# ScottHCL/recommend

Hardware: AMD Instinct MI355X
Metric: ranked samples/sec (fwd+bwd) at B=4096 seq=128; AUC parity vs ref (higher is better)
Workload: dtype f32-emulated (fp16-pair / split-bf16); 1 GPU; C2: OneTrans 4L d128 H4 f512 L_NS12 L_S128 (seq 3x42), Criteo-shape 13 dense + 26 ids, replicated tables, fwd+bwd+optimizer; global_batch=4096, per_gpu_batch=4096, seq_len=128, parallelism=dp1

## Files before the change

include/onetrans_hip.h:

```cpp
#ifndef ONETRANS_HIP_H
#define ONETRANS_HIP_H

#include <stddef.h>
#include <stdint.h>

#ifdef __cplusplus
extern "C" {
#endif

#define OT_OK 0
#define OT_ERR_INVALID_ARG 1
#define OT_ERR_UNSUPPORTED 2
#define OT_ERR_HIP 3

#define OT_GEMM_NN 0
#define OT_GEMM_NT 1

#define OT_AX_NONE 0
#define OT_AX_RMSNORM 1
#define OT_AX_GELU 2
#define OT_AX_BF16 4
#define OT_AX_BF16_RMSNORM 5

#define OT_EPI_BIAS 1
// ... 73 lines not shown
                           float* dW, int64_t dw_gstride, float* db, int64_t db_gstride,
                           int accumulate, void* workspace, size_t ws_bytes, const float* a_bound,
                           const float* d_bound, int precision, void* stream);

int ot_transpose_banks(const float* src, float* dst, const int64_t* banks_dev, int nbanks, int64_t total_tiles,
                       void* stream);

size_t ot_split_image_elems(int G, int N, int K);
int ot_split_images(const float* base, const int64_t* desc_dev, int ndesc, int64_t total_units, uint16_t* img,
                    int precision, void* stream);
int ot_mixed_gemm_img(int mode, const float* A, int64_t lda, int K, const int32_t* in_rows,
                      int a_xform, const float* a_rstd, const float* a_gamma,
                      const float* W, int64_t w_gstride, int64_t ldw, int N,
                      const int32_t* tile_group, int ntiles,
                      const float* bias, int64_t bias_gstride,
                      float* C, int64_t ldc, const int32_t* out_rows, int epi,
                      const float* res, int64_t ldres, int res_tok,
                      const float* aux, int64_t ldaux,
                      uint32_t seed, uint32_t site, float drop_rate, int tail_K, int tail_I,
                      const int32_t* tail_pos, const uint16_t* b_image, int image_ntn, int image_tn0,
                      int precision, void* stream);
int ot_plane_wide(int on);
int ot_wgrad_wide(int on);
int ot_mixed_gemm_rms_img(int mode, const float* A, int64_t lda, int K, const int32_t* in_rows,
                          int a_xform, const float* a_rstd, const float* a_gamma,
                          const float* W, int64_t w_gstride, int64_t ldw, int N,
                          const int32_t* tile_group, int ntiles,
                          const float* bias, int64_t bias_gstride,
                          float* C, int64_t ldc, const int32_t* out_rows, int epi,
                          const float* res, int64_t ldres, int res_tok,
                          const float* aux, int64_t ldaux,
                          uint32_t seed, uint32_t site, float drop_rate, int tail_K, int tail_I,
                          const int32_t* tail_pos, const ot_rms_epilogue* rms, const uint16_t* b_image,
                          int image_ntn, int image_tn0, int precision, void* stream);

int ot_attn_fwd(const float* qkv, int64_t ld, int B, int H, int I, int K, const int32_t* qpos,
                int head_dim, float* out, float* lse, int precision, void* stream);
size_t ot_attn_fwd_fp8_workspace_size(int B, int H, int I, int head_dim);
int ot_attn_fwd_fp8(const float* qkv, int64_t ld, int B, int H, int I, int K, const int32_t* qpos,
                    int head_dim, float* out, float* lse, void* workspace, size_t ws_bytes, void* stream);
#define OT_FP8_DEQUANT 1
#define OT_FP8_TWO_TERM 2
int ot_attn_fwd_fp8_ex(float* qkv, int64_t ld, int B, int H, int I, int K, const int32_t* qpos, int head_dim,
                       float* out, float* lse, void* workspace, size_t ws_bytes, int flags, void* stream);
int ot_attn_fwd_fp8_deq16(const float* qkv, int64_t ld, int B, int H, int I, int K, const int32_t* qpos,
                          int head_dim, float* out, float* lse, void* workspace, size_t ws_bytes, int flags,
// ... 135 lines not shown
```

recommend_amd/_lib.py:

```python

from __future__ import annotations

import ctypes
import os
from ctypes import c_float, c_int, c_int64, c_size_t, c_uint32, c_void_p, c_char_p

_HERE = os.path.dirname(os.path.abspath(__file__))
LIB_PATH = os.environ.get('ONETRANS_HIP_LIB') or os.path.join(_HERE, 'libonetrans_hip.so')
HEADER = os.path.join(os.path.dirname(_HERE), 'include', 'onetrans_hip.h')

OT_GEMM_NN, OT_GEMM_NT = 0, 1
OT_AX_NONE, OT_AX_RMSNORM, OT_AX_GELU, OT_AX_BF16, OT_AX_BF16_RMSNORM = 0, 1, 2, 4, 5
OT_EPI_BIAS, OT_EPI_GELU_BWD, OT_EPI_GELU = 1, 2, 4
OT_EPI_DROPOUT, OT_EPI_RESIDUAL, OT_EPI_ACCUMULATE = 8, 16, 32
OT_EPI_ROW_RSTD, OT_EPI_RMSNORM_BWD, OT_EPI_ROWDOT = 64, 128, 256
OT_EPI_C_BF16 = 512
OT_EPI_AUX_BF16 = 1024
OT_ATTN_DQKV_BF16 = 1
OT_ATTN_QKV_BF16 = 2
OT_ATTN_DQ_PART_BF16 = 4
OT_WG_D_BF16 = 8
OT_MATMUL_F32, OT_MATMUL_SPLIT_BF16, OT_MATMUL_BF16 = 0, 1, 2
OT_FP8_DEQUANT, OT_FP8_TWO_TERM = 1, 2
MATMUL_MODES = {'f32': OT_MATMUL_F32, 'split': OT_MATMUL_SPLIT_BF16, 'bf16': OT_MATMUL_BF16}
# ... 24 lines not shown
    'ot_gemm_tile_rows': (c_int, []),
    'ot_mixed_gemm': (c_int, [c_int, P, I64, c_int, P, c_int, P, P, P, I64, I64, c_int, P, c_int, P, I64,
                              P, I64, P, c_int, P, I64, c_int, P, I64, c_uint32, c_uint32, c_float, c_int,
                              c_int, P, c_int, P]),
    'ot_mixed_gemm_rms_workspace_size': (c_size_t, [c_int, c_int]),
    'ot_mixed_gemm_rms': (c_int, [c_int, P, I64, c_int, P, c_int, P, P, P, I64, I64, c_int, P, c_int, P, I64,
                                  P, I64, P, c_int, P, I64, c_int, P, I64, c_uint32, c_uint32, c_float, c_int,
                                  c_int, P, P, c_int, P]),
    'ot_wgrad_workspace_size': (c_size_t, [c_int, c_int, c_int]),
    'ot_mixed_gemm_wgrad': (c_int, [P, I64, P, c_int, P, P, P, I64, P, c_int, c_int, P, c_int, P, c_int, P,
                                    I64, P, I64, c_int, P, c_size_t, c_int, P]),
    'ot_mixed_gemm_wgrad_ex': (c_int, [P, I64, P, c_int, P, P, P, I64, P, c_int, c_int, P, c_int, P, c_int, P,
                                       I64, P, I64, c_int, P, c_size_t, P, P, c_int, P]),
    'ot_transpose_banks': (c_int, [P, P, P, c_int, I64, P]),
    'ot_mixed_gemm_img': (c_int, [c_int, P, I64, c_int, P, c_int, P, P, P, I64, I64, c_int, P, c_int, P, I64,
                                  P, I64, P, c_int, P, I64, c_int, P, I64, c_uint32, c_uint32, c_float, c_int,
                                  c_int, P, P, c_int, c_int, c_int, P]),
    'ot_mixed_gemm_rms_img': (c_int, [c_int, P, I64, c_int, P, c_int, P, P, P, I64, I64, c_int, P, c_int, P, I64,
                                      P, I64, P, c_int, P, I64, c_int, P, I64, c_uint32, c_uint32, c_float, c_int,
                                      c_int, P, P, P, c_int, c_int, c_int, P]),
    'ot_split_image_elems': (c_size_t, [c_int, c_int, c_int]),
    'ot_plane_wide': (c_int, [c_int]),
    'ot_wgrad_wide': (c_int, [c_int]),
    'ot_split_images': (c_int, [P, P, c_int, I64, P, c_int, P]),
    'ot_attn_fwd': (c_int, [P, I64, c_int, c_int, c_int, c_int, P, c_int, P, P, c_int, P]),
    'ot_attn_fwd_fp8_workspace_size': (c_size_t, [c_int, c_int, c_int, c_int]),
    'ot_attn_fwd_fp8': (c_int, [P, I64, c_int, c_int, c_int, c_int, P, c_int, P, P, P, c_size_t, P]),
    'ot_attn_fwd_fp8_ex': (c_int, [P, I64, c_int, c_int, c_int, c_int, P, c_int, P, P, P, c_size_t, c_int, P]),
    'ot_attn_fwd_fp8_deq16': (c_int, [P, I64, c_int, c_int, c_int, c_int, P, c_int, P, P, P, c_size_t, c_int, P, P]),
    'ot_attn_bwd_workspace_size': (c_size_t, [c_int, c_int, c_int]),
    'ot_attn_bwd': (c_int, [P, I64, P, P, P, c_int, c_int, c_int, c_int, P, c_int, P, P, c_int, P]),
    'ot_attn_bwd_ex_workspace_size': (c_size_t, [c_int, c_int, c_int, c_int, c_int, c_int, c_int]),
    'ot_attn_bwd_ex': (c_int, [P, I64, P, P, P, c_int, c_int, c_int, c_int, P, c_int, P, P, c_size_t, c_int, P]),
    'ot_attn_bwd_dqkv_bf16_supported': (c_int, [c_int, c_int, c_int, c_int, c_int]),
    'ot_attn_bwd_bf16_forms': (c_int, [c_int, c_int, c_int, c_int, c_int]),
    'ot_attn_slice_supported': (c_int, [c_int, c_int, c_int, c_int]),
    'ot_attn_bwd_flags_workspace_size': (c_size_t, [c_int, c_int, c_int, c_int, c_int, c_int, c_int, c_int]),
    'ot_attn_bwd_flags': (c_int, [P, I64, P, P, P, c_int, c_int, c_int, c_int, P, c_int, P, c_int, P, c_size_t, c_int, P]),
    'ot_attn_fwd_cached': (c_int, [P, I64, P, I64, P, c_int, c_int, c_int, c_int, c_int, c_int, P, P]),
    'ot_attn_amax_supported': (c_int, [c_int, c_int, c_int, c_int, c_int]),
    'ot_attn_fwd_amax': (c_int, [P, I64, c_int, c_int, c_int, c_int, P, c_int, P, P, P, P, c_int, P]),
    'ot_attn_bwd_amax': (c_int, [P, I64, P, P, P, c_int, c_int, c_int, c_int, P, c_int, P, P, c_size_t, P, P, c_int,
                                 P]),
    'ot_pyramid_select': (c_int, [P, c_float, c_int, c_int, c_int, c_int, P, P, P, c_int, P]),
    'ot_rmsnorm_fwd': (c_int, [P, I64, P, P, I64, P, I64, c_int, c_float, P]),
    'ot_rmsnorm_bwd_workspace_size': (c_size_t, [I64, c_int]),
# ... 89 lines not shown
```

recommend_amd/csrc/gemm.hip:

```cpp
#include <algorithm>
#include <cstdlib>
#include <atomic>
#include <mutex>

#include "common.h"

namespace ot {

#ifndef OT_GEMM_BK
#define OT_GEMM_BK 16
#endif
#ifndef OT_GEMM_MINWG
#define OT_GEMM_MINWG 3
#endif
#ifndef OT_GEMM_PRIO
#define OT_GEMM_PRIO 0
#endif
#ifndef OT_GEMM_RMS_EARLY
#define OT_GEMM_RMS_EARLY 1
#endif
#ifndef OT_PLANE_BF16_NSTG
#define OT_PLANE_BF16_NSTG 3
#endif
constexpr int PLANE_BF16_NSTG = OT_PLANE_BF16_NSTG;
// ... 33 lines not shown
  const int32_t* tile_group;
  const float* bias; int64_t bias_gstride;
  float* C; int64_t ldc; const int32_t* out_rows;
  int epi;
  const float* res; int64_t ldres; int res_tok;
  const float* aux; int64_t ldaux;
  uint32_t seed, site, drop_thr; float drop_scale; int tail_K, tail_I; int drop_width;
  int ntm, ntn;
  float* rstd_out; float eps;
  const float* nx; int64_t ldnx; const float* ngamma; const float* nrstd;
  const float* dres; int64_t lddres; int dres_K, dres_I; const int32_t* dres_inv;
  float* dxm; int64_t lddxm; float* dgpart;
  float* rowpart;
  float* rowdot; int rowdot_n;
  uint16_t* gelu_out; int64_t ldgelu;
  const int32_t* tail_pos;
  const uint16_t* bimg; int bimg_ntn, bimg_tn0;
  uint16_t* xn_out; int64_t ldxn;
  uint16_t* c16_out; int64_t ldc16;
  float* rowmax_out; int rowmax_n;
  const float* a_rowmax; int a_rowmax_n;
  float* amax_out;
  float* rowabs_out; int rowabs_n;
};

__device__ __forceinline__ float row32_max(float v) {
  v = fmaxf(v, __int_as_float(__builtin_amdgcn_update_dpp(0, __float_as_int(v), 0xB1, 0xF, 0xF, false)));
  v = fmaxf(v, __int_as_float(__builtin_amdgcn_update_dpp(0, __float_as_int(v), 0x4E, 0xF, 0xF, false)));
  v = fmaxf(v, __int_as_float(__builtin_amdgcn_update_dpp(0, __float_as_int(v), 0x141, 0xF, 0xF, false)));
  v = fmaxf(v, __int_as_float(__builtin_amdgcn_update_dpp(0, __float_as_int(v), 0x140, 0xF, 0xF, false)));
  const auto a = __builtin_amdgcn_permlane16_swap(__float_as_uint(v), __float_as_uint(v), false, false);
  return fmaxf(__uint_as_float(a[0]), __uint_as_float(a[1]));
}
__device__ __forceinline__ float row32_sum(float v) {
#pragma unroll
  for (int o = 16; o > 0; o >>= 1) v += __shfl_xor(v, o, 64);
  return v;
}

__device__ __forceinline__ f32x4 apply_pro(f32x4 v, int xf, float rs, const float* gamma, int k) {
  if (xf == OT_AX_RMSNORM) {
    v.x *= rs * gamma[k]; v.y *= rs * gamma[k + 1]; v.z *= rs * gamma[k + 2]; v.w *= rs * gamma[k + 3];
  } else if (xf == OT_AX_GELU) {
    v = gelu_erf4(v);
  }
  return v;
// ... 9 lines not shown
    rem = b % per_chunk;
    return true;
  }
  const int x = b & 7, j = b >> 3;
  c = x + 8 * (j / per_chunk);
  rem = j % per_chunk;
  return c < nchunks;
}

__device__ __forceinline__ void store_out4(float* dst, f32x4 v) {
  if (OT_GEMM_NT_STORE) __builtin_nontemporal_store(v, reinterpret_cast<f32x4*>(dst));
  else *reinterpret_cast<f32x4*>(dst) = v;
}
#ifndef OT_GEMM_NT_STORE16
#define OT_GEMM_NT_STORE16 1
#endif
__device__ __forceinline__ void store_out4_bf16(uint16_t* dst, f32x4 v) {
  if (OT_GEMM_NT_STORE16) __builtin_nontemporal_store(bf16_rne4(v), reinterpret_cast<u32x2*>(dst));
  else *reinterpret_cast<u32x2*>(dst) = bf16_rne4(v);
}

template <int EPIT, int LAYOUT, bool ROWSCALE, int RBN = 8, bool GS = false>
__device__ __forceinline__ void gemm_vec_epilogue(const GemmArgs& p, const f32x16* acc, float* smem, int tm,
                                                  int n0, int g, int sub = 0, int tid = -1) {
  const int epi = EPIT;
  const int t = tid >= 0 ? tid : (int)threadIdx.x, lane = t & 63, wave = t >> 6;
  const int h = lane >> 5, li = lane & 31;
    constexpr int CLD = GT + 4;
    static_assert(64 * CLD + 8 * GT <= 4 * GT * GLD, "epilogue LDS exceeds the staging buffers");
    float* ct = smem;
    const int c4 = t & 31, rb = t >> 5;
    const int col = n0 + 4 * c4;
    f32x4 bias4 = {0.f, 0.f, 0.f, 0.f};
    if (epi & OT_EPI_BIAS) bias4 = *reinterpret_cast<const f32x4*>(p.bias + (int64_t)g * p.bias_gstride + col);
    const bool need_tok = (epi & OT_EPI_DROPOUT) || ((epi & OT_EPI_RESIDUAL) && p.res_tok);
    constexpr bool RMSBWD = EPIT >= 0 && (EPIT & OT_EPI_RMSNORM_BWD);
    constexpr bool ROWRSTD = EPIT >= 0 && (EPIT & OT_EPI_ROW_RSTD);
    constexpr bool ROWDOT = EPIT >= 0 && (EPIT & OT_EPI_ROWDOT);
    constexpr bool GSTORE = GS && (EPIT == OT_EPI_BIAS || EPIT == (OT_EPI_BIAS | OT_EPI_C_BF16));
    constexpr bool CBF = EPIT >= 0 && (EPIT & OT_EPI_C_BF16);
    constexpr bool AUXBF = EPIT >= 0 && (EPIT & OT_EPI_AUX_BF16);
    f32x4 rdb4 = {0.f, 0.f, 0.f, 0.f};
    if (ROWDOT) rdb4 = *reinterpret_cast<const f32x4*>(p.bias + (int64_t)g * p.bias_gstride + col);
    float* dgs = ct + 64 * CLD;
    f32x4 ngam = {0.f, 0.f, 0.f, 0.f};
    if (RMSBWD) {
      ngam = *reinterpret_cast<const f32x4*>(p.ngamma + col);
      *reinterpret_cast<f32x4*>(dgs + rb * GT + 4 * c4) = f32x4{0.f, 0.f, 0.f, 0.f};
    }
    constexpr int RB = RMSBWD ? RBN / 2 : RBN;
    float am = 0.f;
#pragma unroll
    for (int hf = 0; hf < 2; ++hf) {
      int orow[8];
      float rsc[8];
#pragma unroll
      for (int i = 0; i < 8; ++i) {
        const int lr = rb + 8 * i;
        const int64_t gr = (int64_t)tm * GT + (LAYOUT == 0 ? (lr >> 5) * 64 + 32 * hf + (lr & 31) : 64 * hf + lr);
        orow[i] = p.out_rows ? p.out_rows[gr] : (int)gr;
        if (ROWSCALE) {
          const int ir = p.in_rows ? p.in_rows[gr] : (int)gr;
          rsc[i] = ir >= 0 ? p.a_rstd[ir] : 0.f;
        }
      }
      if (LAYOUT == 0) {
#pragma unroll
        for (int n = 0; n < 2; ++n)
#pragma unroll
          for (int r = 0; r < 16; ++r)
            ct[((wave >> 1) * 32 + (r & 3) + 8 * (r >> 2) + 4 * h) * CLD + (wave & 1) * 64 + 32 * n + li] = acc[2 * hf + n][r];
      } else if (LAYOUT == 1) {
        if ((wave >> 1) == hf) {
#pragma unroll
          for (int nb = 0; nb < 4; ++nb)
#pragma unroll
            for (int r = 0; r < 16; ++r)
              ct[((wave & 1) * 32 + (r & 3) + 8 * (r >> 2) + 4 * h) * CLD + 32 * nb + li] = acc[nb][r];
        }
      } else if (LAYOUT == 4) {
        if ((wave >> 1) == sub) {
#pragma unroll
// ... 489 lines not shown
        }
        crow[col] = v;
      }
    }
  }
}

__global__ __launch_bounds__(256) void row_rstd_finish_kernel(const float* __restrict__ part, int ntn,
                                                              const int32_t* __restrict__ out_rows, int64_t nrows,
                                                              int N, float eps, float* rstd_out) {
  const int64_t gr = (int64_t)blockIdx.x * blockDim.x + threadIdx.x;
  if (gr >= nrows) return;
  const int orr = out_rows ? out_rows[gr] : (int)gr;
  if (orr < 0) return;
  float s = 0.f;
  for (int j = 0; j < ntn; ++j) s += part[gr * ntn + j];
  rstd_out[orr] = rsqrtf(s / (float)N + eps);
}

constexpr int PG_A_BYTES = GT * 16 * 4;
constexpr int PG_B_BYTES = 3 * GT * 16 * 2;
constexpr int PG_STG_BYTES = PG_A_BYTES + PG_B_BYTES;
static_assert(64 * (GT + 4) * 4 + 8 * GT * 4 <= 2 * PG_STG_BYTES, "plane GEMM epilogue LDS");

typedef __attribute__((address_space(3))) void lds_void_t;

template <int TERMS>
constexpr int pg_stage_bytes() { return PG_A_BYTES + (TERMS == 1 ? GT * 16 * 2 : PG_B_BYTES); }

constexpr uint32_t PAIR_IMAGE_TAG = 0x7FC17FC1u;

template <int AXT, int EPIT, int NSTG, int MINW, int TERMS = 6>
__global__ __launch_bounds__(256, MINW) void plane_gemm_kernel(GemmArgs p) {
  static_assert(NSTG >= 2 && NSTG <= 4, "plane GEMM stages");
  static_assert(TERMS == 6 || TERMS == 1 || (TERMS == 2 && (AXT == OT_AX_RMSNORM || AXT == OT_AX_GELU || AXT == OT_AX_NONE)),
                "plane GEMM terms");
  constexpr bool ABF = AXT == OT_AX_BF16 || AXT == OT_AX_BF16_RMSNORM;
  constexpr bool RSC = AXT == OT_AX_RMSNORM || AXT == OT_AX_BF16_RMSNORM;
  static_assert(!ABF || TERMS == 1, "bf16 A operands go with OT_MATMUL_BF16");
  constexpr int STG = pg_stage_bytes<TERMS>();
  extern __shared__ __attribute__((aligned(16))) float smem[];
  char* lds = reinterpret_cast<char*>(smem);
  const int nwg = p.ntm * p.ntn;
  const int wg = xcd_remap(blockIdx.x, nwg);
  const int tm = wg / p.ntn, tn = wg % p.ntn;
  const int g = p.tile_group ? p.tile_group[tm] : 0;
// ... 57 lines not shown
  const int aoff0 = ra * 64 + 16 * ((2 * h) ^ ((li >> 2) & 3));
  const int aoff1 = ra * 64 + 16 * ((2 * h + 1) ^ ((li >> 2) & 3));
  const int boff = PG_A_BYTES + li * 32 + 16 * (h ^ ((li >> 3) & 1));
  const int aoffb = ra * 32 + 16 * (h ^ ((li >> 3) & 1));

  bool xnw = false;
  float xrs = 0.f;
  uint16_t* xnp = nullptr;
  float* gsm = reinterpret_cast<float*>(lds + NSTG * STG);
  constexpr bool XN = RSC && TERMS == 1;
  if (XN && p.xn_out && tn == 0) {
    for (int k = 4 * t; k < p.K; k += 4 * 256)
      *reinterpret_cast<f32x4*>(gsm + k) = *reinterpret_cast<const f32x4*>(p.a_gamma + k);
    const int64_t xgr = (int64_t)tm * GT + ra;
    const int xir = p.in_rows ? p.in_rows[xgr] : (int)xgr;
    xnw = xir >= 0;
    if (xnw) {
      xrs = p.a_rstd[xir];
      xnp = p.xn_out + (int64_t)xir * p.ldxn + 8 * h;
    }
  }

  float abound = 1.f;
  if constexpr (TERMS == 2) {
    const int64_t gr = (int64_t)tm * GT + ra;
    int ir = p.in_rows ? p.in_rows[gr] : (int)gr;
    ir = ir < 0 ? 0 : ir;
    if constexpr (AXT == OT_AX_RMSNORM) {
      abound = p.a_rstd[ir];
    } else {
      abound = AXT == OT_AX_GELU ? 0.17f : 0.f;
      for (int j = 0; j < p.a_rowmax_n; ++j) abound = fmaxf(abound, p.a_rowmax[(int64_t)ir * p.a_rowmax_n + j]);
    }
  }
  issue(0, 0);
  if (NSTG >= 3 && nk > 1) issue(1, 1);
  if (NSTG >= 4 && nk > 2) issue(2, 2);
  float asc = 1.f, ainv = 1.f;
  if constexpr (TERMS == 2) {
    asc = pow2_scale14(AXT == OT_AX_RMSNORM ? sqrtf((float)p.K) / abound : abound);
    ainv = 1.f / asc;
  }
  for (int kt = 0; kt < nk; ++kt) {
    constexpr int OPS = ABF ? 2 : (TERMS == 1 ? 3 : 2 + BPL);
    const int ahead = (NSTG - 2 < nk - 1 - kt) ? NSTG - 2 : nk - 1 - kt;
    if (ahead >= 2) asm volatile("s_waitcnt vmcnt(%0)" :: "n"(2 * OPS) : "memory");
    else if (ahead == 1) asm volatile("s_waitcnt vmcnt(%0)" :: "n"(OPS) : "memory");
    else asm volatile("s_waitcnt vmcnt(0)" ::: "memory");
    asm volatile("s_waitcnt lgkmcnt(0)" ::: "memory");
    __builtin_amdgcn_s_barrier();
    asm volatile("" ::: "memory");
    if (kt + NSTG - 1 < nk) issue(kt + NSTG - 1, (kt + NSTG - 1) % NSTG);
    const char* sb = lds + (kt % NSTG) * STG;
    u32x4 fb[4][3];
#pragma unroll
    for (int nb = 0; nb < 4; ++nb)
#pragma unroll
      for (int q = 0; q < (TERMS == 1 ? 1 : BPL); ++q)
        fb[nb][q] = *reinterpret_cast<const u32x4*>(sb + boff + q * 4096 + nb * 1024);
    if constexpr (ABF) {
      u32x4 fa[3];
      fa[0] = *reinterpret_cast<const u32x4*>(sb + aoffb);
      if (XN && xnw) {
        const float* gp = gsm + 16 * kt + 8 * h;
// ... 31 lines not shown
#pragma unroll
      for (int nb = 0; nb < 4; ++nb) acc[nb] = mfma_pair(fa, fb[nb], acc[nb]);
    } else {
      split8t<TERMS == 1 ? 1 : 6>(av, fa);
#pragma unroll
      for (int nb = 0; nb < 4; ++nb) acc[nb] = mfma_terms<TERMS == 1 ? 1 : 6>(fa, fb[nb], acc[nb]);
    }
  }
  if constexpr (TERMS == 2) {
    const float* csc = reinterpret_cast<const float*>(bimg0 + 2 * GT * 16 * 2);
    const float bad = reinterpret_cast<const uint32_t*>(csc)[GT] == PAIR_IMAGE_TAG ? 1.f : __builtin_nanf("");
    float cinv[4];
#pragma unroll
    for (int nb = 0; nb < 4; ++nb) cinv[nb] = bad / csc[32 * nb + li];
#pragma unroll
    for (int r = 0; r < 16; ++r) {
      const float ri = __shfl(ainv, (r & 3) + 8 * (r >> 2) + 4 * h, 64);
#pragma unroll
      for (int nb = 0; nb < 4; ++nb) acc[nb][r] *= ri * cinv[nb];
    }
  }
  asm volatile("s_waitcnt vmcnt(0) lgkmcnt(0)" ::: "memory");
  __syncthreads();
  gemm_vec_epilogue<EPIT, 1, RSC, MINW >= 4 ? OT_PLANE_EPI_RBN : 8, TERMS == 1>(p, acc, smem, tm, n0, g);
}

#ifndef OT_PLANE_WIDE
#define OT_PLANE_WIDE 1
#endif
#ifndef OT_PLANE_WIDE_WL
#define OT_PLANE_WIDE_WL 2
#endif
constexpr int PW_COLS = 2 * GT;
template <int AXT>
constexpr bool pw_abf() { return AXT == OT_AX_BF16 || AXT == OT_AX_BF16_RMSNORM; }
template <int AXT>
constexpr int pw_abytes() { return pw_abf<AXT>() ? GT * 32 : GT * 64; }
template <int AXT>
constexpr int pw_sub() { return pw_abytes<AXT>() + 2 * GT * 32; }
template <int AXT>
constexpr int pw_nstg() { return pw_abf<AXT>() ? 3 : 2; }
template <int AXT>
constexpr int pw_stage_lds() { return pw_nstg<AXT>() * 2 * pw_sub<AXT>(); }

template <int AXT, int EPIT, int WL = OT_PLANE_WIDE_WL>
__global__ __launch_bounds__(256, 2) void plane_wide_kernel(GemmArgs p) {
  static_assert(AXT == OT_AX_NONE || pw_abf<AXT>(), "wide plane GEMM: A in f32 (rounded) or bf16");
// ... 491 lines not shown
  X(OT_AX_BF16_RMSNORM, 0)                                                                     \
  X(OT_AX_BF16_RMSNORM, OT_EPI_BIAS)                                                           \
  X(OT_AX_BF16_RMSNORM, OT_EPI_BIAS | OT_EPI_C_BF16)                                           \
  X(OT_AX_BF16, 0)                                                                             \
  X(OT_AX_BF16, OT_EPI_BIAS | OT_EPI_RESIDUAL)                                                 \
  X(OT_AX_BF16, OT_EPI_BIAS | OT_EPI_RESIDUAL | OT_EPI_DROPOUT)                                \
  X(OT_AX_BF16, OT_EPI_BIAS | OT_EPI_RESIDUAL | OT_EPI_DROPOUT | OT_EPI_ROW_RSTD)              \
  X(OT_AX_BF16, OT_EPI_BIAS | OT_EPI_RESIDUAL | OT_EPI_ROW_RSTD)                               \
  X(OT_AX_BF16, OT_EPI_GELU_BWD | OT_EPI_ROWDOT | OT_EPI_C_BF16 | OT_EPI_AUX_BF16)             \
  X(OT_AX_BF16, OT_EPI_GELU_BWD | OT_EPI_ROWDOT | OT_EPI_C_BF16)                               \
  X(OT_AX_BF16, OT_EPI_RMSNORM_BWD | OT_EPI_DROPOUT)                                           \
  X(OT_AX_BF16, OT_EPI_RMSNORM_BWD)

static int plane_tile_auto(int K, int N, int ntiles) {
  (void)ntiles;
  return N <= K ? 1 : 0;
}

static std::atomic<int> g_plane_wide{OT_PLANE_WIDE};
extern "C" int ot_plane_wide(int on) {
  const int prev = g_plane_wide.load();
  if (on >= 0) g_plane_wide.store(on > 4 ? 4 : on);
  return prev;
}

static void (*plane_wide_for(int x, int e, int kind, int* stage_lds))(GemmArgs) {
  void (*k)(GemmArgs) = nullptr;
#define OT_WIDE_PICK(AX_, EP_)                                                                        \
  if (x == (AX_) && e == (EP_)) {                                                                     \
    k = kind == 3 ? plane_sq_kernel<AX_, EP_> : kind == 2 ? plane_big_kernel<AX_, EP_> : plane_wide_kernel<AX_, EP_>; \
    *stage_lds = kind == 3 ? ps_stage_lds<AX_>() : kind == 2 ? pb_stage_lds<AX_>() : pw_stage_lds<AX_>();  \
  }
  OT_WIDE_LIST(OT_WIDE_PICK)
#undef OT_WIDE_PICK
  static std::once_flag once;
  std::call_once(once, [] {
#define OT_WIDE_ATTR(AX_, EP_)                                                                               \
  (void)hipFuncSetAttribute((const void*)plane_wide_kernel<AX_, EP_>, hipFuncAttributeMaxDynamicSharedMemorySize, \
                            pw_stage_lds<AX_>() + 4096);                                                         \
  (void)hipFuncSetAttribute((const void*)plane_big_kernel<AX_, EP_>, hipFuncAttributeMaxDynamicSharedMemorySize,  \
                            pb_stage_lds<AX_>() + 4096);                                                        \
  (void)hipFuncSetAttribute((const void*)plane_sq_kernel<AX_, EP_>, hipFuncAttributeMaxDynamicSharedMemorySize,   \
                            ps_stage_lds<AX_>() + 4096);
    OT_WIDE_LIST(OT_WIDE_ATTR)
#undef OT_WIDE_ATTR
    (void)hipGetLastError();
// ... 1206 lines not shown
      p.dgpart = dgpart;
    }
  }
  if (epi & OT_EPI_DROPOUT) {
    OT_REQUIRE(drop_rate >= 0.f && drop_rate < 1.f, "ot_mixed_gemm: drop_rate out of range");
    p.drop_thr = drop_threshold(drop_rate);
    p.drop_scale = 1.f / (1.f - drop_rate);
  }
  const bool split = prec != OT_MATMUL_F32 && mode == OT_GEMM_NT;
  const bool one = prec == OT_MATMUL_BF16;
  const size_t shmem = split ? 4 * GT * SRS * sizeof(uint16_t) : 4 * GT * GLD * sizeof(float);
  auto a16 = [](const void* q) { return ((uintptr_t)q & 15) == 0; };
  const bool vec_ok = ldc % 4 == 0 && a16(C) && (!(epi & OT_EPI_RESIDUAL) || (ldres % 4 == 0 && a16(res))) &&
                      (!(epi & OT_EPI_GELU_BWD) || (ldaux % 4 == 0 && a16(aux))) &&
                      (!(epi & (OT_EPI_BIAS | OT_EPI_ROWDOT)) || (bias_gstride % 4 == 0 && a16(bias)));
  const bool edge = (K % GBK) != 0 || (N % GT) != 0 || !vec_ok;
  OT_REQUIRE(!rms_flags || !edge, "ot_mixed_gemm_rms: needs K %% %d == 0 and 16-B aligned operands", GBK);
  const unsigned nwg = (unsigned)ntiles * p.ntn;
  hipStream_t s = (hipStream_t)stream;
  void (*kern)(GemmArgs) = nullptr;
  bool plane = false;
  int wide_lds = 0;
  int wide_kind = 0;
  const int e = epi, x = a_xform;
#define OT_SPEC(NT_, AX_, EP_)                                                                  \
  if (mode == (NT_ ? OT_GEMM_NT : OT_GEMM_NN) && x == AX_ && e == (EP_))                         \
    kern = split ? (one ? (edge ? mixed_gemm_kernel<NT_, AX_, EP_, true, 1> : mixed_gemm_kernel<NT_, AX_, EP_, false, 1>) \
                        : (edge ? mixed_gemm_kernel<NT_, AX_, EP_, true, SPLIT_TERMS>                         \
                                : mixed_gemm_kernel<NT_, AX_, EP_, false, SPLIT_TERMS>))                      \
                 : (edge ? mixed_gemm_kernel<NT_, AX_, EP_, true, 0> : mixed_gemm_kernel<NT_, AX_, EP_, false, 0>);
  OT_SPEC(true, OT_AX_RMSNORM, 0)
  OT_SPEC(true, OT_AX_RMSNORM, OT_EPI_BIAS)
  OT_SPEC(true, OT_AX_GELU, OT_EPI_BIAS | OT_EPI_RESIDUAL | OT_EPI_DROPOUT)
  OT_SPEC(true, OT_AX_GELU, OT_EPI_BIAS | OT_EPI_RESIDUAL)
  OT_SPEC(true, OT_AX_NONE, OT_EPI_RESIDUAL | OT_EPI_DROPOUT)
  OT_SPEC(true, OT_AX_NONE, OT_EPI_RESIDUAL)
  OT_SPEC(true, OT_AX_NONE, OT_EPI_BIAS)
  OT_SPEC(true, OT_AX_NONE, OT_EPI_GELU_BWD)
  OT_SPEC(true, OT_AX_NONE, OT_EPI_GELU_BWD | OT_EPI_ROWDOT)
  OT_SPEC(true, OT_AX_NONE, 0)
  OT_SPEC(true, OT_AX_NONE, OT_EPI_ACCUMULATE)
  OT_SPEC(true, OT_AX_NONE, OT_EPI_RESIDUAL | OT_EPI_DROPOUT | OT_EPI_ROW_RSTD)
  OT_SPEC(true, OT_AX_NONE, OT_EPI_RESIDUAL | OT_EPI_ROW_RSTD)
  OT_SPEC(true, OT_AX_GELU, OT_EPI_BIAS | OT_EPI_RESIDUAL | OT_EPI_DROPOUT | OT_EPI_ROW_RSTD)
  OT_SPEC(true, OT_AX_GELU, OT_EPI_BIAS | OT_EPI_RESIDUAL | OT_EPI_ROW_RSTD)
  OT_SPEC(true, OT_AX_NONE, OT_EPI_RMSNORM_BWD)
// ... 36 lines not shown
    if (one && x == OT_AX_NONE && e == (OT_EPI_GELU_BWD | OT_EPI_C_BF16 | OT_EPI_AUX_BF16))
      pk = plane_gemm_kernel<OT_AX_NONE, OT_EPI_GELU_BWD | OT_EPI_C_BF16 | OT_EPI_AUX_BF16, PLANE_BF16_NSTG, 4, 1>;
    if (one && x == OT_AX_NONE && e == (OT_EPI_GELU_BWD | OT_EPI_ROWDOT | OT_EPI_AUX_BF16))
      pk = plane_gemm_kernel<OT_AX_NONE, OT_EPI_GELU_BWD | OT_EPI_ROWDOT | OT_EPI_AUX_BF16, PLANE_BF16_NSTG, 4, 1>;
    if (one && x == OT_AX_RMSNORM && e == (OT_EPI_BIAS | OT_EPI_C_BF16))
      pk = plane_gemm_kernel<OT_AX_RMSNORM, OT_EPI_BIAS | OT_EPI_C_BF16, PLANE_BF16_NSTG, 4, 1>;
#define OT_PSPEC_BF(EP_) if (one && x == OT_AX_BF16 && e == (EP_)) pk = plane_gemm_kernel<OT_AX_BF16, EP_, PLANE_BF16_NSTG, 4, 1>;
    OT_PSPEC_BF(OT_EPI_BIAS | OT_EPI_RESIDUAL | OT_EPI_DROPOUT)
    OT_PSPEC_BF(OT_EPI_BIAS | OT_EPI_RESIDUAL)
    OT_PSPEC_BF(OT_EPI_BIAS | OT_EPI_RESIDUAL | OT_EPI_DROPOUT | OT_EPI_ROW_RSTD)
    OT_PSPEC_BF(OT_EPI_BIAS | OT_EPI_RESIDUAL | OT_EPI_ROW_RSTD)
    OT_PSPEC_BF(OT_EPI_RMSNORM_BWD)
    OT_PSPEC_BF(OT_EPI_RMSNORM_BWD | OT_EPI_DROPOUT)
    OT_PSPEC_BF(0)
    OT_PSPEC_BF(OT_EPI_GELU_BWD | OT_EPI_ROWDOT | OT_EPI_C_BF16 | OT_EPI_AUX_BF16)
    OT_PSPEC_BF(OT_EPI_GELU_BWD | OT_EPI_ROWDOT | OT_EPI_C_BF16)
#undef OT_PSPEC_BF
#define OT_PSPEC_BR(EP_) if (one && x == OT_AX_BF16_RMSNORM && e == (EP_)) pk = plane_gemm_kernel<OT_AX_BF16_RMSNORM, EP_, PLANE_BF16_NSTG, 4, 1>;
    OT_PSPEC_BR(0)
    OT_PSPEC_BR(OT_EPI_BIAS)
    OT_PSPEC_BR(OT_EPI_BIAS | OT_EPI_C_BF16)
#undef OT_PSPEC_BR
    if (pk) { kern = pk; plane = true; }
    const int wmode = g_plane_wide.load(std::memory_order_relaxed);
    if (pk && one && wmode && N % PW_COLS == 0 && K % 32 == 0 && !(p.xn_out && K > 1024)) {
      int kind = wmode == 1 ? plane_tile_auto(K, N, ntiles) : wmode - 1;
      if (kind == 2 && N % PB_COLS != 0) kind = 1;
      if (kind == 3 && ntiles % 2 != 0) kind = 1;
      int stage_lds = 0;
      void (*wk)(GemmArgs) = kind ? plane_wide_for(x, e, kind, &stage_lds) : nullptr;
      if (wk) {
        kern = wk;
        wide_lds = stage_lds;
        wide_kind = kind;
      }
    }
  }
  OT_REQUIRE((x != OT_AX_BF16 && x != OT_AX_BF16_RMSNORM) || plane,
             "ot_mixed_gemm: no plane GEMM for a_xform %d with epilogue %d (or edge tiles)", x, epi);
  OT_REQUIRE(!p.c16_out || (plane && one && p.ldc16 % 4 == 0 && ((uintptr_t)p.c16_out % 8) == 0 &&
                            !(epi & (OT_EPI_RMSNORM_BWD | OT_EPI_C_BF16))),
             "ot_mixed_gemm_rms: c16_out needs the bf16-mode plane GEMM (not with OT_EPI_RMSNORM_BWD / C_BF16), "
             "ldc16 %% 4 == 0 and 8-B alignment");
  OT_REQUIRE(!(epi & (OT_EPI_C_BF16 | OT_EPI_AUX_BF16)) || plane,
             "ot_mixed_gemm: OT_EPI_C_BF16 / OT_EPI_AUX_BF16 need the bf16-mode plane GEMM with OT_EPI_GELU_BWD "
             "[| OT_EPI_ROWDOT] or OT_EPI_BIAS alone (epilogue %d)", epi);
// ... 27 lines not shown
    else if (mode == OT_GEMM_NT && split)
      kern = edge ? mixed_gemm_kernel<true, -1, -1, true, SPLIT_TERMS> : mixed_gemm_kernel<true, -1, -1, false, SPLIT_TERMS>;
    else if (mode == OT_GEMM_NT)
      kern = edge ? mixed_gemm_kernel<true, -1, -1, true, 0> : mixed_gemm_kernel<true, -1, -1, false, 0>;
    else
      kern = edge ? mixed_gemm_kernel<false, -1, -1, true, 0> : mixed_gemm_kernel<false, -1, -1, false, 0>;
  }
  static std::once_flag lds_once;
  std::call_once(lds_once, [] {
    const int bytes = (int)std::max(4 * GT * GLD * sizeof(float), 4 * GT * SRS * sizeof(uint16_t));
    for (void (*k)(GemmArgs) : {mixed_gemm_kernel<true, -1, -1, true, 0>, mixed_gemm_kernel<true, -1, -1, false, 0>,
                                mixed_gemm_kernel<false, -1, -1, true, 0>, mixed_gemm_kernel<false, -1, -1, false, 0>,
                                mixed_gemm_kernel<true, -1, -1, true, SPLIT_TERMS>,
                                mixed_gemm_kernel<true, -1, -1, false, SPLIT_TERMS>,
                                mixed_gemm_kernel<true, -1, -1, true, 1>, mixed_gemm_kernel<true, -1, -1, false, 1>})
      (void)hipFuncSetAttribute((const void*)k, hipFuncAttributeMaxDynamicSharedMemorySize, bytes);
    (void)hipGetLastError();
  });
  if (wide_lds > 0) {
    const size_t wshm = std::max((size_t)wide_lds + xn_lds, (size_t)(64 * (GT + 4) + 8 * GT) * 4);
    const unsigned wg = wide_kind == 3 ? (unsigned)(ntiles / 2) * (unsigned)(N / PW_COLS)
                                       : (unsigned)ntiles * (unsigned)(N / (wide_kind == 2 ? PB_COLS : PW_COLS));
    hipLaunchKernelGGL(kern, dim3(wg), dim3(wide_kind == 3 ? 512 : 256), wshm, s, p);
  } else {
    hipLaunchKernelGGL(kern, dim3(nwg), dim3(256), launch_shmem, s, p);
  }
  OT_LAUNCH_CHECK("ot_mixed_gemm");
  if (dgpart) {
    launch_colsum_reduce(dgpart, ntiles, N, rms->dgamma, rms->accumulate_dgamma, s, dgpart + (int64_t)ntiles * N);
    OT_LAUNCH_CHECK("ot_mixed_gemm_rms(dgamma)");
  }
  if (p.rowpart) {
    const int64_t nr = (int64_t)ntiles * GT;
    hipLaunchKernelGGL(row_rstd_finish_kernel, dim3(ceil_div(nr, 256)), dim3(256), 0, s, p.rowpart, p.ntn, out_rows,
                       nr, N, rms->eps, rms->rstd_out);
    OT_LAUNCH_CHECK("ot_mixed_gemm_rms(rstd)");
  }
  return OT_OK;
}

extern "C" int ot_mixed_gemm(int mode, const float* A, int64_t lda, int K, const int32_t* in_rows,
                             int a_xform, const float* a_rstd, const float* a_gamma,
                             const float* W, int64_t w_gstride, int64_t ldw, int N,
                             const int32_t* tile_group, int ntiles,
                             const float* bias, int64_t bias_gstride,
                             float* C, int64_t ldc, const int32_t* out_rows, int epi,
// ... 236 lines not shown
```

recommend_amd/kernels.py:

```python

from __future__ import annotations

import contextlib
import ctypes
import functools
import os
import threading
from typing import Optional, Tuple, Union

import torch

from . import _lib
from ._lib import call, size

Ptrish = Union[None, torch.Tensor, Tuple[torch.Tensor, int]]


class Probe:

    def __init__(self):
        self.recs = []

    def begin(self):
        ev = torch.cuda.Event(enable_timing=True)
# ... 249 lines not shown
        _probe.end('mixed_gemm', 2.0 * m_rows * K * N, ev, f'wgrad ax{a_xform} M{m_rows} K{K} N{N} ch{nchunks}',
                   (2.0 if (a_xform & ~_lib.OT_WG_D_BF16) == _lib.OT_AX_BF16 else 4.0) * m_rows * K
                   + (2.0 if a_xform & _lib.OT_WG_D_BF16 else 4.0) * m_rows * N
                   + 4.0 * m_rows * ((a_xform & ~_lib.OT_WG_D_BF16) == _lib.OT_AX_RMSNORM) + 4.0 * ngroups * K * N,
                   wterms)


def transpose_banks(src, dst, banks_dev, nbanks, total_tiles) -> None:
    call('ot_transpose_banks', ptr(src), ptr(dst), ptr(banks_dev), nbanks, total_tiles, stream())


def split_image_elems(G: int, N: int, K: int) -> int:
    return int(_lib.load().ot_split_image_elems(G, N, K))


def plane_wide(on: int = -1) -> int:
    return _lib.size('ot_plane_wide', int(on))


def wgrad_wide(on: int = -1) -> int:
    return _lib.size('ot_wgrad_wide', int(on))


def split_images(base, desc_dev, ndesc, total_units, img) -> None:
    call('ot_split_images', ptr(base), ptr(desc_dev), ndesc, total_units, ptr(img), _prec(), stream())


def attn_fwd(qkv: torch.Tensor, ld: int, B: int, H: int, I: int, K: int, hd: int, out: torch.Tensor,
             lse: torch.Tensor, qpos: Optional[torch.Tensor] = None, fp8: bool = False,
             dequant: bool = False, fp8_terms: int = 1, deq16: Optional[torch.Tensor] = None,
             amax: Optional[torch.Tensor] = None, rowmax: Optional[torch.Tensor] = None) -> None:
    if fp8 and fp8_terms not in (1, 2):
        raise ValueError(f'fp8_terms {fp8_terms}: 1 or 2')
    ws = None
    if fp8:
        ws = workspace(size('ot_attn_fwd_fp8_workspace_size', B, H, I, hd), qkv.device)
    ev = _probe.begin() if _probe is not None else None
    if fp8 and deq16 is not None:
        call('ot_attn_fwd_fp8_deq16', ptr(qkv), ld, B, H, I, K, ptr(qpos), hd, ptr(out), ptr(lse), ptr(ws),
             ws.numel(), _lib.OT_FP8_TWO_TERM if fp8_terms == 2 else 0, ptr(deq16), stream())
    elif fp8:
        call('ot_attn_fwd_fp8_ex', ptr(qkv), ld, B, H, I, K, ptr(qpos), hd, ptr(out), ptr(lse), ptr(ws),
             ws.numel(), (_lib.OT_FP8_DEQUANT if dequant else 0) | (_lib.OT_FP8_TWO_TERM if fp8_terms == 2 else 0),
             stream())
    elif amax is not None or rowmax is not None:
        call('ot_attn_fwd_amax', ptr(qkv), ld, B, H, I, K, ptr(qpos), hd, ptr(out), ptr(lse), ptr(amax), ptr(rowmax),
# ... 255 lines not shown
```

Baseline: 197,000 samples/s.

## Add panel plane GEMM kernel and LDS-cached row metadata for epilogue

```diff
diff --git a/include/onetrans_hip.h b/include/onetrans_hip.h
--- a/include/onetrans_hip.h
+++ b/include/onetrans_hip.h
@@ -119,6 +119,9 @@
                       int precision, void* stream);
 int ot_plane_wide(int on);
 int ot_wgrad_wide(int on);
+int ot_plane_rowmeta(int on);
+int ot_plane_panel(int on);
+int ot_plane_panel_launches(void);
 int ot_mixed_gemm_rms_img(int mode, const float* A, int64_t lda, int K, const int32_t* in_rows,
                           int a_xform, const float* a_rstd, const float* a_gamma,
                           const float* W, int64_t w_gstride, int64_t ldw, int N,
diff --git a/recommend_amd/_lib.py b/recommend_amd/_lib.py
--- a/recommend_amd/_lib.py
+++ b/recommend_amd/_lib.py
@@ -70,6 +70,9 @@
     'ot_split_image_elems': (c_size_t, [c_int, c_int, c_int]),
     'ot_plane_wide': (c_int, [c_int]),
     'ot_wgrad_wide': (c_int, [c_int]),
+    'ot_plane_rowmeta': (c_int, [c_int]),
+    'ot_plane_panel': (c_int, [c_int]),
+    'ot_plane_panel_launches': (c_int, []),
     'ot_split_images': (c_int, [P, P, c_int, I64, P, c_int, P]),
     'ot_attn_fwd': (c_int, [P, I64, c_int, c_int, c_int, c_int, P, c_int, P, P, c_int, P]),
     'ot_attn_fwd_fp8_workspace_size': (c_size_t, [c_int, c_int, c_int, c_int]),
diff --git a/recommend_amd/csrc/gemm.hip b/recommend_amd/csrc/gemm.hip
--- a/recommend_amd/csrc/gemm.hip
+++ b/recommend_amd/csrc/gemm.hip
@@ -79,6 +79,8 @@
   const float* a_rowmax; int a_rowmax_n;
   float* amax_out;
   float* rowabs_out; int rowabs_n;
+  int rowmeta;
+  int panel_w;
 };
 
 __device__ __forceinline__ float row32_max(float v) {
@@ -134,7 +136,8 @@
 
 template <int EPIT, int LAYOUT, bool ROWSCALE, int RBN = 8, bool GS = false>
 __device__ __forceinline__ void gemm_vec_epilogue(const GemmArgs& p, const f32x16* acc, float* smem, int tm,
-                                                  int n0, int g, int sub = 0, int tid = -1) {
+                                                  int n0, int g, int sub = 0, int tid = -1,
+                                                  const int* rmeta = nullptr) {
   const int epi = EPIT;
   const int t = tid >= 0 ? tid : (int)threadIdx.x, lane = t & 63, wave = t >> 6;
   const int h = lane >> 5, li = lane & 31;
@@ -170,6 +173,11 @@
       for (int i = 0; i < 8; ++i) {
         const int lr = rb + 8 * i;
         const int64_t gr = (int64_t)tm * GT + (LAYOUT == 0 ? (lr >> 5) * 64 + 32 * hf + (lr & 31) : 64 * hf + lr);
+        if (LAYOUT == 1 && rmeta) {
+          orow[i] = rmeta[64 * hf + lr];
+          if (ROWSCALE) rsc[i] = __int_as_float(rmeta[GT + 64 * hf + lr]);
+          continue;
+        }
         orow[i] = p.out_rows ? p.out_rows[gr] : (int)gr;
         if (ROWSCALE) {
           const int ir = p.in_rows ? p.in_rows[gr] : (int)gr;
@@ -705,6 +713,10 @@
 constexpr int PG_B_BYTES = 3 * GT * 16 * 2;
 constexpr int PG_STG_BYTES = PG_A_BYTES + PG_B_BYTES;
 static_assert(64 * (GT + 4) * 4 + 8 * GT * 4 <= 2 * PG_STG_BYTES, "plane GEMM epilogue LDS");
+constexpr int PG_META_OFF = 64 * (GT + 4) * 4 + 8 * GT * 4;
+constexpr int PG_META_BYTES = 2 * GT * 4;
+static_assert(PG_META_OFF >= PG_STG_BYTES + PG_A_BYTES + 2 * GT * 16 * 2 && PG_META_OFF + PG_META_BYTES <= 2 * PG_STG_BYTES,
+              "plane GEMM row metadata LDS");
 
 typedef __attribute__((address_space(3))) void lds_void_t;
 
@@ -808,9 +820,14 @@
   }
 
   float abound = 1.f;
+  constexpr bool PMETA = TERMS == 2 && AXT != OT_AX_GELU;
+  int mrow = 0;
+  bool mok = false;
   if constexpr (TERMS == 2) {
     const int64_t gr = (int64_t)tm * GT + ra;
     int ir = p.in_rows ? p.in_rows[gr] : (int)gr;
+    mok = ir >= 0;
+    if (PMETA && p.rowmeta) mrow = p.out_rows ? p.out_rows[gr] : (int)gr;
     ir = ir < 0 ? 0 : ir;
     if constexpr (AXT == OT_AX_RMSNORM) {
       abound = p.a_rstd[ir];
@@ -823,9 +840,18 @@
   if (NSTG >= 3 && nk > 1) issue(1, 1);
   if (NSTG >= 4 && nk > 2) issue(2, 2);
   float asc = 1.f, ainv = 1.f;
+  const int* rmeta = nullptr;
   if constexpr (TERMS == 2) {
     asc = pow2_scale14(AXT == OT_AX_RMSNORM ? sqrtf((float)p.K) / abound : abound);
     ainv = 1.f / asc;
+    if (PMETA && p.rowmeta) {
+      int* rm = reinterpret_cast<int*>(lds + PG_META_OFF);
+      if (h == 0) {
+        rm[ra] = mrow;
+        if (RSC) rm[GT + ra] = __float_as_int(mok ? abound : 0.f);
+      }
+      rmeta = rm;
+    }
   }
   for (int kt = 0; kt < nk; ++kt) {
     constexpr int OPS = ABF ? 2 : (TERMS == 1 ? 3 : 2 + BPL);
@@ -903,7 +929,232 @@
   }
   asm volatile("s_waitcnt vmcnt(0) lgkmcnt(0)" ::: "memory");
   __syncthreads();
-  gemm_vec_epilogue<EPIT, 1, RSC, MINW >= 4 ? OT_PLANE_EPI_RBN : 8, TERMS == 1>(p, acc, smem, tm, n0, g);
+  gemm_vec_epilogue<EPIT, 1, RSC, MINW >= 4 ? OT_PLANE_EPI_RBN : 8, TERMS == 1>(p, acc, smem, tm, n0, g, 0, -1, rmeta);
+}
+
+constexpr int PP_STG = PG_A_BYTES + 2 * GT * 16 * 2;
+constexpr int PP_CLD = GT + 4;
+constexpr int PP_EPI_OFF = 2 * PP_STG;
+constexpr int pp_epi_wave(int SR) { return SR * PP_CLD * 4; }
+constexpr int pp_meta_off(int SR) { return PP_EPI_OFF + 4 * pp_epi_wave(SR); }
+constexpr int pp_lds(int SR) { return pp_meta_off(SR) + PG_META_BYTES; }
+static_assert(3 * pp_lds(8) <= 160 * 1024 && 4 * pp_lds(2) <= 160 * 1024, "panel plane GEMM LDS");
+
+template <int EPIT, bool ROWSCALE, int SR>
+__device__ __forceinline__ void panel_epilogue(const GemmArgs& p, const f32x16* acc, float* ctw, const int* rmeta,
+                                               int row0, int n0, f32x4 bias4, float& am) {
+  static_assert(!(EPIT & ~(OT_EPI_BIAS | OT_EPI_GELU_BWD | OT_EPI_ROWDOT)), "panel plane GEMM epilogue flags");
+  constexpr int epi = EPIT;
+  constexpr bool ROWDOT = (EPIT & OT_EPI_ROWDOT) != 0;
+  const int lane = threadIdx.x & 63, h = lane >> 5, li = lane & 31;
+  const int c4 = li, col = n0 + 4 * c4;
+  const f32x4 rdb4 = bias4;
+  constexpr int HQ = SR / 2;
+  static_assert(SR == 8 || SR == 2, "panel epilogue slice rows");
+#pragma unroll
+  for (int j = 0; j < 16 / HQ; ++j) {
+#pragma unroll
+    for (int nb = 0; nb < 4; ++nb)
+#pragma unroll
+      for (int q = 0; q < HQ; ++q) ctw[(q + HQ * h) * PP_CLD + 32 * nb + li] = acc[nb][HQ * j + q];
+    int orow[HQ];
+    float rsc[HQ];
+#pragma unroll
+    for (int i = 0; i < HQ; ++i) {
+      const int sr = h + 2 * i, r = HQ * j + sr % HQ;
+      const int tr = row0 + (r & 3) + 8 * (r >> 2) + 4 * (sr / HQ);
+      orow[i] = rmeta[tr];
+      if (ROWSCALE) rsc[i] = __int_as_float(rmeta[GT + tr]);
+    }
+    f32x4 aux4[HQ];
+#pragma unroll
+    for (int i = 0; i < HQ; ++i) {
+      const int64_t o = orow[i] < 0 ? 0 : orow[i];
+      if (epi & OT_EPI_GELU_BWD) aux4[i] = *reinterpret_cast<const f32x4*>(p.aux + o * p.ldaux + col);
+    }
+    asm volatile("s_waitcnt lgkmcnt(0)" ::: "memory");
+#pragma unroll
+    for (int i = 0; i < HQ; ++i) {
+      const int orr = orow[i];
+      f32x4 v = *reinterpret_cast<const f32x4*>(ctw + (h + 2 * i) * PP_CLD + 4 * c4);
+      if (ROWSCALE) v = v * rsc[i];
+      if (epi & OT_EPI_BIAS) v += bias4;
+      if (p.rowmax_out) {
+        float mx = fmaxf(fmaxf(v.x, v.y), fmaxf(v.z, v.w));
+        mx = row32_max(mx);
+        if (orr >= 0 && c4 == 0) p.rowmax_out[(int64_t)orr * p.rowmax_n + n0 / GT] = mx;
+      }
+      if (epi & OT_EPI_GELU_BWD) {
+        v *= gelu_erf_grad4(aux4[i]);
+        if (p.gelu_out && orr >= 0) {
+          const f32x4 hv = gelu_erf4(aux4[i]);
+          store_out4_bf16(p.gelu_out + (int64_t)orr * p.ldgelu + col, hv);
+        }
+        if (ROWDOT) {
+          const f32x4 ub = aux4[i] - rdb4;
+          const float sd = row32_sum(v.x * ub.x + v.y * ub.y + v.z * ub.z + v.w * ub.w);
+          if (orr >= 0 && c4 == 0) p.rowdot[(int64_t)orr * p.rowdot_n + n0 / GT] = sd;
+        }
+      }
+      if (orr >= 0) store_out4(p.C + (int64_t)orr * p.ldc + col, v);
+      if (orr >= 0) am = amax4(am, v);
+      if (p.rowabs_out) {
+        float mx = amax4(0.f, v);
+        mx = row32_max(mx);
+        if (orr >= 0 && c4 == 0) p.rowabs_out[(int64_t)orr * p.rowabs_n + n0 / GT] = mx;
+      }
+    }
+    asm volatile("s_waitcnt lgkmcnt(0)" ::: "memory");
+  }
+}
+
+template <int AXT, int EPIT, int MINW = 3, int SR = 8, bool HOLDA = false>
+__global__ __launch_bounds__(256, MINW) void plane_panel_kernel(GemmArgs p) {
+  static_assert(AXT == OT_AX_RMSNORM || AXT == OT_AX_NONE, "panel plane GEMM prologues");
+  static_assert(MINW * pp_lds(SR) <= 160 * 1024, "panel plane GEMM LDS per CU");
+  constexpr bool RSC = AXT == OT_AX_RMSNORM;
+  extern __shared__ __attribute__((aligned(16))) float smem[];
+  char* lds = reinterpret_cast<char*>(smem);
+  const int pw = p.panel_w, npan = (p.ntn + pw - 1) / pw;
+  const int wg = xcd_remap(blockIdx.x, p.ntm * npan);
+  const int tm = wg / npan, tnb = (wg % npan) * pw;
+  const int tne = tnb + pw < p.ntn ? tnb + pw : p.ntn;
+  const int g = p.tile_group ? p.tile_group[tm] : 0;
+  const int t = threadIdx.x, lane = t & 63, wave = t >> 6;
+  const int h = lane >> 5, li = lane & 31;
+  const int nk = p.K >> 4;
+
+  const float* asrc[2];
+#pragma unroll
+  for (int i = 0; i < 2; ++i) {
+    const int r = (2 * wave + i) * 16 + (lane >> 2);
+    const int64_t gr = (int64_t)tm * GT + r;
+    int ir = p.in_rows ? p.in_rows[gr] : (int)gr;
+    ir = ir < 0 ? 0 : ir;
+    const int lc = (lane & 3) ^ ((r >> 2) & 3);
+    asrc[i] = p.A + (int64_t)ir * p.lda + 4 * lc;
+  }
+  const int gb = p.w_gstride ? g : 0;
+  const int64_t tstride = (int64_t)nk * PG_B_BYTES;
+  const char* bpan = reinterpret_cast<const char*>(p.bimg) + ((int64_t)gb * p.bimg_ntn + p.bimg_tn0) * tstride;
+  const int blane = 2 * wave * 1024 + 16 * lane;
+  auto issue = [&](int tn, int ks, int buf) {
+    char* sb = lds + buf * PP_STG;
+    const char* bs = bpan + tn * tstride + (int64_t)ks * PG_B_BYTES + blane;
+    if (!HOLDA || tn == tnb) {
+#pragma unroll
+      for (int i = 0; i < 2; ++i)
+        __builtin_amdgcn_global_load_lds((const void*)(asrc[i] + 16 * ks), (lds_void_t*)(sb + (2 * wave + i) * 1024),
+                                         16, 0, 0);
+    }
+#pragma unroll
+    for (int i = 0; i < 2; ++i)
+      __builtin_amdgcn_global_load_lds((const void*)(bs + i * 1024),
+                                       (lds_void_t*)(sb + PG_A_BYTES + (2 * wave + i) * 1024), 16, 0, 0);
+  };
+
+  const int ra = 32 * wave + li;
+  const int aoff0 = ra * 64 + 16 * ((2 * h) ^ ((li >> 2) & 3));
+  const int aoff1 = ra * 64 + 16 * ((2 * h + 1) ^ ((li >> 2) & 3));
+  const int boff = PG_A_BYTES + li * 32 + 16 * (h ^ ((li >> 3) & 1));
+
+  float abound;
+  int mrow;
+  bool mok;
+  {
+    const int64_t gr = (int64_t)tm * GT + ra;
+    int ir = p.in_rows ? p.in_rows[gr] : (int)gr;
+    mok = ir >= 0;
+    mrow = p.out_rows ? p.out_rows[gr] : (int)gr;
+    ir = ir < 0 ? 0 : ir;
+    if constexpr (AXT == OT_AX_RMSNORM) {
+      abound = p.a_rstd[ir];
+    } else {
+      abound = 0.f;
+      for (int j = 0; j < p.a_rowmax_n; ++j) abound = fmaxf(abound, p.a_rowmax[(int64_t)ir * p.a_rowmax_n + j]);
+    }
+  }
+  issue(tnb, 0, 0);
+  if (nk > 1) issue(tnb, 1, 1);
+  const float asc = pow2_scale14(AXT == OT_AX_RMSNORM ? sqrtf((float)p.K) / abound : abound);
+  const float ainv = 1.f / asc;
+  int* rmeta = reinterpret_cast<int*>(lds + pp_meta_off(SR));
+  if (h == 0) {
+    rmeta[ra] = mrow;
+    if (RSC) rmeta[GT + ra] = __float_as_int(mok ? abound : 0.f);
+  }
+  float* ctw = reinterpret_cast<float*>(lds + PP_EPI_OFF + wave * pp_epi_wave(SR));
+  float am = 0.f;
+  u32x4 fah[HOLDA ? 8 : 1][2];
+
+  for (int tn = tnb; tn < tne; ++tn) {
+    const float* csc = reinterpret_cast<const float*>(bpan + tn * tstride + 2 * GT * 16 * 2);
+    float craw[4];
+#pragma unroll
+    for (int nb = 0; nb < 4; ++nb) craw[nb] = csc[32 * nb + li];
+    uint32_t tag = reinterpret_cast<const uint32_t*>(csc)[GT];
+    f32x4 bias4 = {0.f, 0.f, 0.f, 0.f};
+    if (EPIT & (OT_EPI_BIAS | OT_EPI_ROWDOT))
+      bias4 = *reinterpret_cast<const f32x4*>(p.bias + (int64_t)g * p.bias_gstride + tn * GT + 4 * li);
+    f32x16 acc[4];
+#pragma unroll
+    for (int a = 0; a < 4; ++a)
+#pragma unroll
+      for (int r = 0; r < 16; ++r) acc[a][r] = 0.f;
+    auto kstep = [&](int kt) {
+      asm volatile("s_waitcnt vmcnt(0)" ::: "memory");
+      asm volatile("s_waitcnt lgkmcnt(0)" ::: "memory");
+      __builtin_amdgcn_s_barrier();
+      asm volatile("" ::: "memory");
+      if (kt >= 1 && kt + 1 < nk) issue(tn, kt + 1, (kt + 1) & 1);
+      const char* sb = lds + (kt & 1) * PP_STG;
+      u32x4 fb[4][3];
+#pragma unroll
+      for (int nb = 0; nb < 4; ++nb)
+#pragma unroll
+        for (int q = 0; q < 2; ++q) fb[nb][q] = *reinterpret_cast<const u32x4*>(sb + boff + q * 4096 + nb * 1024);
+      u32x4 fa[3];
+      if (!HOLDA || tn == tnb) {
+        const f32x4 a0 = *reinterpret_cast<const f32x4*>(sb + aoff0);
+        const f32x4 a1 = *reinterpret_cast<const f32x4*>(sb + aoff1);
+        const float av[8] = {a0.x, a0.y, a0.z, a0.w, a1.x, a1.y, a1.z, a1.w};
+        pair8(av, asc, fa);
+        if (HOLDA) { fah[kt][0] = fa[0]; fah[kt][1] = fa[1]; }
+      } else {
+        fa[0] = fah[kt][0]; fa[1] = fah[kt][1];
+      }
+#pragma unroll
+      for (int nb = 0; nb < 4; ++nb) acc[nb] = mfma_pair(fa, fb[nb], acc[nb]);
+    };
+    if constexpr (HOLDA) {
+#pragma unroll
+      for (int kt = 0; kt < 8; ++kt) kstep(kt);
+    } else {
+      for (int kt = 0; kt < nk; ++kt) kstep(kt);
+    }
+    asm volatile("" : "+v"(craw[0]), "+v"(craw[1]), "+v"(craw[2]), "+v"(craw[3]), "+v"(tag), "+v"(bias4));
+    {
+      const float bad = tag == PAIR_IMAGE_TAG ? 1.f : __builtin_nanf("");
+      float cinv[4];
+#pragma unroll
+      for (int nb = 0; nb < 4; ++nb) cinv[nb] = bad / craw[nb];
+#pragma unroll
+      for (int r = 0; r < 16; ++r) {
+        const float ri = __shfl(ainv, (r & 3) + 8 * (r >> 2) + 4 * h, 64);
+#pragma unroll
+        for (int nb = 0; nb < 4; ++nb) acc[nb][r] *= ri * cinv[nb];
+      }
+    }
+    if (tn + 1 < tne) {
+      asm volatile("s_waitcnt vmcnt(0) lgkmcnt(0)" ::: "memory");
+      __builtin_amdgcn_s_barrier();
+      asm volatile("" ::: "memory");
+      issue(tn + 1, 0, 0);
+      if (nk > 1) issue(tn + 1, 1, 1);
+    }
+    panel_epilogue<EPIT, RSC, SR>(p, acc, ctw, rmeta, 32 * wave, tn * GT, bias4, am);
+  }
+  if (p.amax_out) amax_flush(p.amax_out, am);
 }
 
 #ifndef OT_PLANE_WIDE
@@ -1441,6 +1692,55 @@
   const int prev = g_plane_wide.load();
   if (on >= 0) g_plane_wide.store(on > 4 ? 4 : on);
   return prev;
+}
+
+#ifndef OT_PLANE_ROWMETA
+#define OT_PLANE_ROWMETA 1
+#endif
+static std::atomic<int> g_plane_rowmeta{OT_PLANE_ROWMETA};
+extern "C" int ot_plane_rowmeta(int on) {
+  const int old = g_plane_rowmeta.load(std::memory_order_relaxed);
+  if (on >= 0) g_plane_rowmeta.store(on ? 1 : 0, std::memory_order_relaxed);
+  return old;
+}
+
+#ifndef OT_PLANE_PANEL
+#define OT_PLANE_PANEL 0
+#endif
+static std::atomic<int> g_plane_panel{OT_PLANE_PANEL};
+extern "C" int ot_plane_panel(int on) {
+  const int old = g_plane_panel.load(std::memory_order_relaxed);
+  if (on >= 0) g_plane_panel.store(on > 299 ? 299 : on, std::memory_order_relaxed);
+  return old;
+}
+static std::atomic<long long> g_plane_panel_launches{0};
+extern "C" int ot_plane_panel_launches(void) {
+  return (int)(g_plane_panel_launches.load(std::memory_order_relaxed) & 0x7fffffff);
+}
+static void (*plane_panel_for(int x, int e, int variant))(GemmArgs) {
+#define OT_PANEL_PICK(AX_, EP_)                                                                          \
+  if (x == (AX_) && e == (EP_))                                                                          \
+    return variant == 2 ? plane_panel_kernel<AX_, EP_, 2, 8, true>                                       \
+         : variant == 1 ? plane_panel_kernel<AX_, EP_, 4, 2, false> : plane_panel_kernel<AX_, EP_, 3, 8, false>;
+  OT_PANEL_PICK(OT_AX_RMSNORM, 0)
+  OT_PANEL_PICK(OT_AX_RMSNORM, OT_EPI_BIAS)
+  OT_PANEL_PICK(OT_AX_NONE, OT_EPI_GELU_BWD)
+  OT_PANEL_PICK(OT_AX_NONE, OT_EPI_GELU_BWD | OT_EPI_ROWDOT)
+#undef OT_PANEL_PICK
+  return nullptr;
+}
+static int plane_panel_width(int ntiles, int ntn) {
+  static const int slots = [] {
+    int dev = 0, cus = 0;
+    if (hipGetDevice(&dev) != hipSuccess ||
+        hipDeviceGetAttribute(&cus, hipDeviceAttributeMultiprocessorCount, dev) != hipSuccess || cus <= 0)
+      cus = 256;
+    return 3 * cus;
+  }();
+  int w = ntn;
+  while (w > 2 && (int64_t)ntiles * ((ntn + w - 1) / w) < 4 * (int64_t)slots) w = (w + 1) / 2;
+  if ((int64_t)ntiles * ((ntn + w - 1) / w) < slots) return 0;
+  return w;
 }
 
 static void (*plane_wide_for(int x, int e, int kind, int* stage_lds))(GemmArgs) {
@@ -2693,6 +2993,7 @@
   bool plane = false;
   int wide_lds = 0;
   int wide_kind = 0;
+  int panel_lds = 0;
   const int e = epi, x = a_xform;
 #define OT_SPEC(NT_, AX_, EP_)                                                                  \
   if (mode == (NT_ ? OT_GEMM_NT : OT_GEMM_NN) && x == AX_ && e == (EP_))                         \
@@ -2775,6 +3076,19 @@
     OT_PSPEC_BR(OT_EPI_BIAS | OT_EPI_C_BF16)
 #undef OT_PSPEC_BR
     if (pk) { kern = pk; plane = true; }
+    p.rowmeta = pk && !one ? g_plane_rowmeta.load(std::memory_order_relaxed) : 0;
+    const bool pair = !one && (x == OT_AX_RMSNORM || (p.a_rowmax && x == OT_AX_NONE));
+    const int pmode = g_plane_panel.load(std::memory_order_relaxed);
+    if (pk && pair && p.ntn >= 2 && pmode) {
+      const int pvar = pmode >= 200 ? (K == 128 ? 2 : 0) : pmode >= 100 ? 1 : 0;
+      const int pwid = pmode == 1 ? plane_panel_width(ntiles, p.ntn) : std::min(std::max(pmode % 100, 2), (int)p.ntn);
+      void (*ppk)(GemmArgs) = pwid > 0 ? plane_panel_for(x, e, pvar) : nullptr;
+      if (ppk) {
+        kern = ppk;
+        p.panel_w = pwid;
+        panel_lds = pp_lds(pvar == 1 ? 2 : 8);
+      }
+    }
     const int wmode = g_plane_wide.load(std::memory_order_relaxed);
     if (pk && one && wmode && N % PW_COLS == 0 && K % 32 == 0 && !(p.xn_out && K > 1024)) {
       int kind = wmode == 1 ? plane_tile_auto(K, N, ntiles) : wmode - 1;
@@ -2848,6 +3162,10 @@
     const unsigned wg = wide_kind == 3 ? (unsigned)(ntiles / 2) * (unsigned)(N / PW_COLS)
                                        : (unsigned)ntiles * (unsigned)(N / (wide_kind == 2 ? PB_COLS : PW_COLS));
     hipLaunchKernelGGL(kern, dim3(wg), dim3(wide_kind == 3 ? 512 : 256), wshm, s, p);
+  } else if (p.panel_w > 0) {
+    const unsigned npan = (unsigned)((p.ntn + p.panel_w - 1) / p.panel_w);
+    hipLaunchKernelGGL(kern, dim3((unsigned)ntiles * npan), dim3(256), (size_t)panel_lds, s, p);
+    g_plane_panel_launches.fetch_add(1, std::memory_order_relaxed);
   } else {
     hipLaunchKernelGGL(kern, dim3(nwg), dim3(256), launch_shmem, s, p);
   }
diff --git a/recommend_amd/kernels.py b/recommend_amd/kernels.py
--- a/recommend_amd/kernels.py
+++ b/recommend_amd/kernels.py
@@ -295,6 +295,18 @@
     return _lib.size('ot_wgrad_wide', int(on))
 
 
+def plane_rowmeta(on: int = -1) -> int:
+    return _lib.size('ot_plane_rowmeta', int(on))
+
+
+def plane_panel(on: int = -1) -> int:
+    return _lib.size('ot_plane_panel', int(on))
+
+
+def plane_panel_launches() -> int:
+    return _lib.size('ot_plane_panel_launches')
+
+
 def split_images(base, desc_dev, ndesc, total_units, img) -> None:
     call('ot_split_images', ptr(base), ptr(desc_dev), ndesc, total_units, ptr(img), _prec(), stream())
 
```

Result: faster. 199,700 samples/s (median of 6 runs) (+1.4%).
